# Vandermode/ELD

Measured on AMD Instinct MI355X. Metric: raw megapixels/sec (noise-synth + U-Net step), higher is better.
Workload: dtype f32; 1 GPU; BASELINE.json configs[1]: full ELD noise model (PGRU, SonyA7S2 params) on 4x1424x2128 packed raw + U-Net fp32 train step (fwd, L1, bwd, Adam), 8 frames per GPU; images_per_gpu=8, global_batch=8, parallelism=dp1

## Files before the change

eld_amd/csrc/conv_wgrad.hip:

```cpp
#include <stdlib.h>
#include "conv.h"

#define TW 32
#define JB 32

typedef __bf16 bf16x8 __attribute__((ext_vector_type(8)));
typedef short s16x4 __attribute__((ext_vector_type(4)));
typedef int i32x4_t __attribute__((ext_vector_type(4)));
typedef _Float16 half8 __attribute__((ext_vector_type(8)));

enum { ALG_F32 = 0, ALG_BFM = 1, ALG_X3 = 2, ALG_H2 = 3 };

template <typename T, int MODE, int WCO, int TH, int ALG>
__global__ __launch_bounds__(256, 2) void wgrad_kernel(const WgradArgs a) {
    constexpr bool BFM = ALG == ALG_BFM, X3 = ALG == ALG_X3, H2 = ALG == ALG_H2;
    static_assert(!(X3 || H2) || sizeof(T) == 4, "x3 / h2: fp32 inputs");
    constexpr int ES = sizeof(T);
    constexpr int EPU = 16 / ES;
    constexpr int LES = X3 ? 6 : (BFM ? 2 : 4);
    constexpr int TAPS = MODE == CONV_3X3 ? 9 : 4;
    constexpr int WPIX = 4 / WCO;
    constexpr int COB = 32 * WCO;
    constexpr int TPIX = TH * TW;
    constexpr int PW = TPIX / WPIX;
    constexpr int KS = PW / 2;
    constexpr int X_PIX = MODE == CONV_3X3 ? (TH + 2) * (TW + 2) : 4 * TPIX;
    extern __shared__ __attribute__((aligned(16))) float lds[];
    constexpr int GROWS = TPIX + ((X3 || H2) ? 1 : 0);
    float* ldsG = lds;
    float* ldsX = lds + GROWS * COB * LES / 4;

    const int tid = threadIdx.x, lane = tid & 63, wave = tid >> 6;
    const int m = lane & 31, hi = lane >> 5;
    const int wco = wave % WCO, wpix = wave / WCO;
    const int IB = a.CA / COB, JBn = a.CBp / JB;
    int bid = xcd_block(a.xcd);
    const int jb = bid % JBn; bid /= JBn;
    const int ib = bid % IB;
    const int ps = bid / IB;
    const int i0 = ib * COB, j0 = jb * JB;
// ... 254 lines not shown
                const int row = (i & 3) + 8 * (i >> 2) + 4 * hi;
                a.part[pbase + ((size_t)t * a.CA + i0 + wco * 32 + row) * a.CBp + j0 + m] = H2 ? acc[t][i] * (1.0f / sc_g) * (1.0f / sc_x) : acc[t][i];
            }
        }
    }
    if (a.bpart && jb == 0) {
        red[wave * 64 + lane] = bsum;
        __syncthreads();
        if (tid < COB) {
            const int wc = tid / 32, mm = tid % 32;
            float s = 0.f;
            for (int wp = 0; wp < WPIX; ++wp) s += red[(wp * WCO + wc) * 64 + mm] + red[(wp * WCO + wc) * 64 + 32 + mm];
            a.bpart[(size_t)ps * a.CA + i0 + tid] = H2 ? s * (1.0f / sc_g) : s;
        }
    }
    if constexpr (XSUM) {
        if (xsum_on) {
            __syncthreads();
            float* r = lds;
#pragma unroll
            for (int e = 0; e < EPU; ++e) r[tid * EPU + e] = xs[e];
            __syncthreads();
            if (tid < JB) {
                constexpr int PARTS = JB / EPU;
                const int part = tid / EPU, comp = tid % EPU;
                float s = 0.f;
                for (int k = 0; k < 256 / PARTS; ++k) s += r[(k * PARTS + part) * EPU + comp];
                a.xbpart[(size_t)ps * a.CBp + j0 + tid] = s;
            }
        }
    }
}

template <typename T, int WCO, int WCI, int WPIX, int TH, int TWT, int STREAM = 0>
__global__ __launch_bounds__(512, 2) void wgrad8_kernel(const WgradArgs a) {
    constexpr int ES = sizeof(T), EPU = 16 / ES, NPC = ES == 4 ? 3 : 1, XQ = 32 / EPU;
    static_assert(WCO * WCI * WPIX == 8, "8 waves");
    constexpr int THREADS = 512, TAPS = 9;
    constexpr int COB = 32 * WCO, JBK = 32 * WCI, TPIX = TH * TWT, PW = TPIX / WPIX, KSB = PW / 16;
    static_assert(TWT == 8 || TWT == 16 || TWT == 32, "tile width");
    static_assert(PW % 16 == 0 && PW >= 16, "a wave's pixel slice is a whole number of 16-pixel k-steps");
    constexpr int X_PIX = (TH + 2) * (TWT + 2);
    constexpr int GBLK = TPIX * 32 + (ES == 4 ? 32 : 0);
    constexpr int GPL = GBLK * WCO, XPL = X_PIX * JBK;
    constexpr int G_Q = COB / EPU, G_UNITS = TPIX * G_Q, G_IT = G_UNITS / THREADS;
    static_assert(G_UNITS % THREADS == 0 && THREADS % G_Q == 0, "a thread stages the same channel quad of G in every iteration");
    constexpr int X_UNITS1 = X_PIX * XQ, X_IT = (X_UNITS1 + THREADS - 1) / THREADS;
    extern __shared__ __attribute__((aligned(16))) float lds[];
    bf16_t* ldsG = reinterpret_cast<bf16_t*>(lds);
    bf16_t* ldsX = ldsG + NPC * GPL;

    const int tid = threadIdx.x, lane = tid & 63, wave = tid >> 6;
    const int m = lane & 31, hi = lane >> 5;
    const int wco = wave % WCO, wci = (wave / WCO) % WCI, wpix = wave / (WCO * WCI);
    const int IB = a.CA / COB, JBn = a.CBp / JBK;
    int bid = xcd_block(a.xcd);
    const int jb = bid % JBn; bid /= JBn;
    const int ib = bid % IB;
    const int ps = bid / IB;
    const int i0 = ib * COB, j0 = jb * JBK;
    const bool do_bias = a.bpart != nullptr && jb == 0;

    f32x16 acc[TAPS];
#pragma unroll
    for (int t = 0; t < TAPS; ++t)
#pragma unroll
        for (int i = 0; i < 16; ++i) acc[t][i] = 0.f;
    float4 bsum4 = make_float4(0.f, 0.f, 0.f, 0.f), bsum4b = make_float4(0.f, 0.f, 0.f, 0.f);

    const int ntiles = a.tiles_x * a.tiles_y;
    const int VP = a.vp;
    const bool seam = VP % TH != 0;
    constexpr unsigned OOB = 0xFFFFFFF0u;
    constexpr int G_STEP = THREADS / G_Q;
    const int g_part = tid % G_Q, g_lp0 = tid / G_Q;
    const int g_px0 = g_lp0 % TWT, g_py0 = g_lp0 / TWT;
    const unsigned g_off0 = (unsigned)(g_px0 * a.CA + i0 + g_part * EPU) * (unsigned)ES;
    const int g_lds0 = ((g_part * EPU) >> 5) * GBLK + g_lp0 * 32 + ((g_part * EPU) & 31);
    auto g_pxy = [&](int it, int& dpx, int& dpy) {
        if (G_STEP >= TWT) { dpx = 0; dpy = it * (G_STEP / TWT); }
        else { dpx = (it * G_STEP) % TWT; dpy = (it * G_STEP) / TWT; }
    };
    const int x_part = (int)((unsigned)tid % (unsigned)XQ);
    int x_hyx[X_IT];
#pragma unroll
    for (int it = 0; it < X_IT; ++it) {
        const int hp = (int)((unsigned)(tid + it * THREADS) / (unsigned)XQ);
        const int hy = hp / (TWT + 2);
        x_hyx[it] = (hy << 8) | (hp - hy * (TWT + 2));
    }
    auto x_alive = [&](int it) { return (it + 1) * THREADS <= X_UNITS1 || (int)((unsigned)(tid + it * THREADS) / (unsigned)XQ) < X_PIX; };
    const char* xs[WCI]; int xC[WCI], xc0[WCI];
#pragma unroll
    for (int cb = 0; cb < WCI; ++cb) {
        const int c = j0 + cb * 32;
        if (c < a.C0) { xs[cb] = static_cast<const char*>(a.x0); xC[cb] = a.C0; xc0[cb] = c; }
        else if (c < a.C0 + a.C1) { xs[cb] = static_cast<const char*>(a.x1); xC[cb] = a.C1; xc0[cb] = c - a.C0; }
        else { xs[cb] = nullptr; xC[cb] = 32; xc0[cb] = 0; }
    }
    float4 rg[G_IT], rx[WCI][X_IT];
// ... 68 lines not shown
        const unsigned y0 = __float_as_uint(r0), y1 = __float_as_uint(r1), y2 = __float_as_uint(r2), y3 = __float_as_uint(r3);
        const unsigned z0 = __float_as_uint(r0 - __uint_as_float(y0 & 0xFFFF0000u)), z1 = __float_as_uint(r1 - __uint_as_float(y1 & 0xFFFF0000u));
        const unsigned z2 = __float_as_uint(r2 - __uint_as_float(y2 & 0xFFFF0000u)), z3 = __float_as_uint(r3 - __uint_as_float(y3 & 0xFFFF0000u));
        auto hp = [](unsigned lo, unsigned hi_) { return __builtin_amdgcn_perm(hi_, lo, 0x07060302u); };
        *reinterpret_cast<uint2*>(d) = make_uint2(hp(x0, x1), hp(x2, x3));
        *reinterpret_cast<uint2*>(d + plane_elems) = make_uint2(hp(y0, y1), hp(y2, y3));
        *reinterpret_cast<uint2*>(d + 2 * plane_elems) = make_uint2(hp(z0, z1), hp(z2, z3));
    };
    auto store_tile = [&]() {
#pragma unroll
        for (int it = 0; it < G_IT; ++it) {
            put3(ldsG + g_lds0 + it * G_STEP * 32, GPL, rg[it]);
            if (do_bias) {
                if constexpr (ES == 4) { bsum4.x += rg[it].x; bsum4.y += rg[it].y; bsum4.z += rg[it].z; bsum4.w += rg[it].w; }
                else {
                    const uint4 q = __builtin_bit_cast(uint4, rg[it]);
                    const float4 lo = unpack_bf4(make_uint2(q.x, q.y)), hi4 = unpack_bf4(make_uint2(q.z, q.w));
                    bsum4.x += lo.x; bsum4.y += lo.y; bsum4.z += lo.z; bsum4.w += lo.w;
                    bsum4b.x += hi4.x; bsum4b.y += hi4.y; bsum4b.z += hi4.z; bsum4b.w += hi4.w;
                }
            }
        }
#pragma unroll
        for (int cb = 0; cb < WCI; ++cb)
#pragma unroll
            for (int it = 0; it < X_IT; ++it)
                if (x_alive(it)) put3(ldsX + (cb * X_PIX + (int)((unsigned)(tid + it * THREADS) / (unsigned)XQ)) * 32 + x_part * EPU, XPL, rx[cb][it]);
    };

    const int gi = lane & 15, gg = lane >> 4;
    constexpr bool ROWSHARE = STREAM == 2;
    static_assert(!ROWSHARE || (NPC == 3 && TWT == 8 && WPIX == 1 && TH % 2 == 0), "row-shared fragments: fp32, 8-pixel-wide tiles, one pixel slice");
    constexpr int HS = TH / 2;
    const int lq0 = ROWSHARE ? HS * TWT * hi + (gi >> 2) : wpix * PW + 8 * hi + (gi >> 2);
    const int pyq = lq0 / TWT, pxq = lq0 - pyq * TWT;
    const bf16_t* gq = ldsG + wco * GBLK + lq0 * 32 + (gg & 1) * 16 + (gi & 3) * 4;
    const bf16_t* xq = ldsX + (wci * X_PIX + pyq * (TWT + 2) + pxq) * 32 + (gg & 1) * 16 + (gi & 3) * 4;
    auto tr8 = [](const bf16_t* p0) {
        const s16x4 lo = __builtin_amdgcn_ds_read_tr16_b64_v4i16((__attribute__((address_space(3))) s16x4*)p0);
        const s16x4 hi4 = __builtin_amdgcn_ds_read_tr16_b64_v4i16((__attribute__((address_space(3))) s16x4*)(p0 + 4 * 32));
        return __builtin_bit_cast(bf16x8, __builtin_shufflevector(lo, hi4, 0, 1, 2, 3, 4, 5, 6, 7));
    };

    if (ps < ntiles) load_tile(ps);
    for (int tile = ps; tile < ntiles; tile += a.psplit) {
        __syncthreads();
        store_tile();
        __syncthreads();
        if (tile + a.psplit < ntiles) load_tile(tile + a.psplit);
        if constexpr (ROWSHARE) {
            constexpr int GI[6] = {0, 1, 2, 0, 1, 0};
            constexpr int XI[6] = {2, 1, 0, 1, 0, 0};
            constexpr int NU = (HS + 2) * 3;
            bf16x8 gr[3][3], xf[2][3];
            auto readG = [&](int s_, bf16x8 (&g3)[3]) {
#pragma unroll
                for (int pc = 0; pc < 3; ++pc) g3[pc] = tr8(gq + pc * GPL + s_ * TWT * 32);
            };
            auto readF = [&](int a_, int kx, bf16x8 (&x3)[3]) {
#pragma unroll
                for (int pc = 0; pc < 3; ++pc) x3[pc] = tr8(xq + pc * XPL + (a_ * (TWT + 2) + kx) * 32);
            };
            readG(0, gr[0]);
            readF(0, 0, xf[0]);
#pragma unroll
            for (int u = 0; u < NU; ++u) {
                const int a_ = u / 3, kx = u % 3;
                if (u + 1 < NU) readF((u + 1) / 3, (u + 1) % 3, xf[(u + 1) & 1]);
                __builtin_amdgcn_sched_barrier(0);
#pragma unroll
// ... 13 lines not shown
            }
        } else
        if constexpr (NPC == 3 && STREAM == 1) {
            constexpr int GI[6] = {0, 1, 2, 0, 1, 0};
            constexpr int XI[6] = {2, 1, 0, 1, 0, 0};
            constexpr int NBLK = KSB * TAPS;
            bf16x8 ga[2][3], xb[2][3];
            auto readG = [&](int ks, bf16x8 (&g3)[3]) {
#pragma unroll
                for (int pc = 0; pc < 3; ++pc) g3[pc] = tr8(gq + pc * GPL + ks * 16 * 32);
            };
            auto readX = [&](int ks, int t, bf16x8 (&x3)[3]) {
                const int lrel = ks * 16, dy0 = lrel / TWT, dxp = lrel - dy0 * TWT;
                const int xoff = (dy0 + t / 3) * (TWT + 2) + dxp + t % 3;
#pragma unroll
                for (int pc = 0; pc < 3; ++pc) x3[pc] = tr8(xq + pc * XPL + xoff * 32);
            };
            readG(0, ga[0]);
            readX(0, 0, xb[0]);
#pragma unroll
            for (int b = 0; b < NBLK; ++b) {
                const int ks = b / TAPS, t = b % TAPS;
                if (b + 1 < NBLK) {
                    const int ks1 = (b + 1) / TAPS, t1 = (b + 1) % TAPS;
                    readX(ks1, t1, xb[(b + 1) & 1]);
                    if (ks1 != ks) readG(ks1, ga[ks1 & 1]);
                }
                __builtin_amdgcn_sched_barrier(0);
#pragma unroll
                for (int q = 0; q < 6; ++q) acc[t] = __builtin_amdgcn_mfma_f32_32x32x16_bf16(ga[ks & 1][GI[q]], xb[b & 1][XI[q]], acc[t], 0, 0, 0);
                __builtin_amdgcn_sched_barrier(0);
            }
        } else
#pragma unroll
        for (int ks = 0; ks < KSB; ++ks) {
            const int lrel = ks * 16;
            const int dy0 = lrel / TWT, dxp = lrel - dy0 * TWT;
            bf16x8 ga[NPC];
#pragma unroll
            for (int pc = 0; pc < NPC; ++pc) ga[pc] = tr8(gq + pc * GPL + lrel * 32);
#pragma unroll
            for (int t0 = 0; t0 < TAPS; t0 += 3) {
                bf16x8 xb[3][NPC];
#pragma unroll
                for (int tt = 0; tt < 3; ++tt) {
                    const int xoff = (dy0 + t0 / 3) * (TWT + 2) + dxp + tt;
#pragma unroll
                    for (int pc = 0; pc < NPC; ++pc) xb[tt][pc] = tr8(xq + pc * XPL + xoff * 32);
                }
                if constexpr (NPC == 3) {
                    constexpr int GI[6] = {0, 1, 2, 0, 1, 0};
                    constexpr int XI[6] = {2, 1, 0, 1, 0, 0};
#pragma unroll
                    for (int q = 0; q < 6; ++q)
#pragma unroll
                        for (int tt = 0; tt < 3; ++tt)
                            acc[t0 + tt] = __builtin_amdgcn_mfma_f32_32x32x16_bf16(ga[GI[q]], xb[tt][XI[q]], acc[t0 + tt], 0, 0, 0);
                } else {
#pragma unroll
                    for (int tt = 0; tt < 3; ++tt) acc[t0 + tt] = __builtin_amdgcn_mfma_f32_32x32x16_bf16(ga[0], xb[tt][0], acc[t0 + tt], 0, 0, 0);
                }
                __builtin_amdgcn_sched_barrier(0);
            }
        }
    }

    __syncthreads();
    float* red = lds;
    const size_t pbase = (size_t)ps * TAPS * a.CA * a.CBp;
    const int wt = wci * WCO + wco;
#pragma unroll
    for (int t = 0; t < TAPS; ++t) {
        if (WPIX > 1) {
            if (wpix > 0) {
#pragma unroll
                for (int i = 0; i < 16; ++i) red[(((wpix - 1) * (WCO * WCI) + wt) * 16 + i) * 64 + lane] = acc[t][i];
            }
            __syncthreads();
            if (wpix == 0) {
                for (int w = 0; w < WPIX - 1; ++w)
#pragma unroll
                    for (int i = 0; i < 16; ++i) acc[t][i] += red[((w * (WCO * WCI) + wt) * 16 + i) * 64 + lane];
            }
            __syncthreads();
        }
        if (wpix == 0) {
#pragma unroll
            for (int i = 0; i < 16; ++i) {
                const int row = (i & 3) + 8 * (i >> 2) + 4 * hi;
                a.part[pbase + ((size_t)t * a.CA + i0 + wco * 32 + row) * a.CBp + j0 + wci * 32 + m] = acc[t][i];
            }
        }
    }
    if (do_bias) {
        __syncthreads();
        if constexpr (ES == 4) reinterpret_cast<float4*>(red)[tid] = bsum4;
        else { reinterpret_cast<float4*>(red)[2 * tid] = bsum4; reinterpret_cast<float4*>(red)[2 * tid + 1] = bsum4b; }
        __syncthreads();
        if (tid < COB) {
            const int q = tid / EPU, comp = tid % EPU;
            float s_ = 0.f;
            for (int k = 0; k < THREADS / G_Q; ++k) s_ += red[(q + k * G_Q) * EPU + comp];
            a.bpart[(size_t)ps * a.CA + i0 + tid] = s_;
        }
    }
}

__device__ __forceinline__ void wg_dma16(i32x4_t rsrc, unsigned voff, unsigned lds_dst) {
    unsigned keep;
    asm volatile("s_nop 4\n\ts_mov_b32 %0, m0\n\ts_mov_b32 m0, %3\n\ts_nop 0\n\tbuffer_load_dwordx4 %1, %2, 0 offen lds\n\ts_mov_b32 m0, %0"
                 : "=&s"(keep) : "v"(voff), "s"(rsrc), "s"(lds_dst) : "memory");
}

template <int WCO, int WCI, int WPIX, int TH, int TWT>
__global__ __launch_bounds__(512, 2) void wgrad8d_kernel(const WgradArgs a) {
    static_assert(WCO * WCI * WPIX == 8, "8 waves");
    static_assert(TWT == 8 || TWT == 16 || TWT == 32, "tile width");
    constexpr int WAVES = 8, THREADS = 512, TAPS = 9;
    constexpr int COB = 32 * WCO, JBK = 32 * WCI, TPIX = TH * TWT, PW = TPIX / WPIX, KSB = PW / 16;
    static_assert(PW % 16 == 0 && PW >= 16, "a wave's pixel slice is a whole number of 16-pixel k-steps");
    constexpr int HW = TWT + 2, X_PIX = (TH + 2) * HW;
    static_assert((TPIX * 4) % 64 == 0, "a block of G is whole DMA pieces");
    constexpr int GB_PIECES = TPIX * 4 / 64, XB_PIECES = (X_PIX * 4 + 63) / 64;
// ... 169 lines not shown
            __syncthreads();
            if (wpix == 0) {
                for (int w = 0; w < WPIX - 1; ++w)
#pragma unroll
                    for (int i = 0; i < 16; ++i) acc[t][i] += red[((w * (WCO * WCI) + wt) * 16 + i) * 64 + lane];
            }
            __syncthreads();
        }
        if (wpix == 0) {
#pragma unroll
            for (int i = 0; i < 16; ++i) {
                const int row = (i & 3) + 8 * (i >> 2) + 4 * hi;
                a.part[pbase + ((size_t)t * a.CA + i0 + wco * 32 + row) * a.CBp + j0 + wci * 32 + m] = acc[t][i];
            }
        }
    }
    if (do_bias) {
        __syncthreads();
        reinterpret_cast<float4*>(red)[2 * tid] = bsum4; reinterpret_cast<float4*>(red)[2 * tid + 1] = bsum4b;
        __syncthreads();
        if (tid < COB) {
            const int q = tid / 8, comp = tid % 8;
            float s_ = 0.f;
            for (int k = 0; k < THREADS / G_Q; ++k) s_ += red[(q + k * G_Q) * 8 + comp];
            a.bpart[(size_t)ps * a.CA + i0 + tid] = s_;
        }
    }
}

static int wgrad8_dma() {
    static const int on = [] { const char* e = getenv("ELD_WGRAD_DMA"); return e ? (int)(atoi(e) != 0) : 1; }();
    return on && !(debug_kernel_mask(-1) & 16);
}
template <int DUMMY>
__global__ __launch_bounds__(512, 2) void wgradt8_kernel(const WgradArgs a) {
    constexpr int WCO = 4, WCI = 2, TH = 8, TWT = 8, TPIX = TH * TWT, THREADS = 512, TAPS = 4, NPC = 3;
    constexpr int COB = 32 * WCO, JBK = 32 * WCI, KSB = TPIX / 16;
    constexpr int GBLK = TPIX * 32 + 32;
    constexpr int GPL = GBLK * WCO, X_PIX = TAPS * TPIX, XPL = X_PIX * JBK;
    constexpr int G_IT = TPIX * (COB / 4) / THREADS, X_IT = X_PIX * 8 / THREADS;
    extern __shared__ __attribute__((aligned(16))) float lds[];
    bf16_t* ldsG = reinterpret_cast<bf16_t*>(lds);
    bf16_t* ldsX = ldsG + NPC * GPL;
    const int tid = threadIdx.x, lane = tid & 63, wave = tid >> 6;
    const int m = lane & 31, hi = lane >> 5;
    const int wco = wave % WCO, wci = wave / WCO;
    const int IB = a.CA / COB, JBn = a.CBp / JBK;
    int bid = xcd_block(a.xcd);
    const int jb = bid % JBn; bid /= JBn;
    const int ib = bid % IB;
    const int ps = bid / IB;
    const int i0 = ib * COB, j0 = jb * JBK;
    const bool xsum_on = a.xbpart != nullptr && ib == 0;
    const int Wx = 2 * a.W, CB = a.C0;

    f32x16 acc[TAPS];
#pragma unroll
    for (int t = 0; t < TAPS; ++t)
#pragma unroll
        for (int i = 0; i < 16; ++i) acc[t][i] = 0.f;
    float4 xs4[WCI];
#pragma unroll
    for (int cb = 0; cb < WCI; ++cb) xs4[cb] = make_float4(0.f, 0.f, 0.f, 0.f);

    const int tiles_per_img = a.tiles_x * a.tiles_y, ntiles = tiles_per_img * a.N;
    constexpr unsigned OOB = 0xFFFFFFF0u;
    const int g_part = tid & 31, g_lp0 = tid >> 5, x_part = tid & 7, x_lp = tid >> 3;
    const int x_py = x_lp / TWT, x_px = x_lp - x_py * TWT;
    float4 rg[G_IT], rx[WCI][X_IT];
    const size_t g_img = (size_t)a.H * a.W * a.CA * 4, x_img = (size_t)4 * a.H * a.W * CB * 4;
    auto load_tile = [&](int tile) {
        const int img = tile / tiles_per_img;
        int ty, tx;
        band_tile(tile - img * tiles_per_img, a.tiles_x, a.tiles_y, a.band, ty, tx);
        const int y0 = ty * TH, x0 = tx * TWT;
        const __amdgpu_buffer_rsrc_t rs_g = __builtin_amdgcn_make_buffer_rsrc((void*)(static_cast<const char*>(a.g) + (size_t)img * g_img), 0, (int)g_img, 0x00020000);
        const __amdgpu_buffer_rsrc_t rs_x = __builtin_amdgcn_make_buffer_rsrc((void*)(static_cast<const char*>(a.x0) + (size_t)img * x_img), 0, (int)x_img, 0x00020000);
#pragma unroll
        for (int it = 0; it < G_IT; ++it) {
            const int lp = g_lp0 + 16 * it, py = lp / TWT, px = lp - py * TWT;
            const int gy = y0 + py, gx = x0 + px;
            const unsigned off = (gy < a.H && gx < a.W) ? (unsigned)(((gy * a.W + gx) * a.CA + i0 + g_part * 4) * 4) : OOB;
            rg[it] = __builtin_bit_cast(float4, __builtin_amdgcn_raw_buffer_load_b128(rs_g, (int)off, 0, 0));
        }
        const bool pok = y0 + x_py < a.H && x0 + x_px < a.W;
#pragma unroll
        for (int cb = 0; cb < WCI; ++cb)
#pragma unroll
            for (int it = 0; it < X_IT; ++it) {
                const int gy = 2 * (y0 + x_py) + (it >> 1), gx = 2 * (x0 + x_px) + (it & 1);
                const unsigned off = pok ? (unsigned)(((gy * Wx + gx) * CB + j0 + cb * 32 + x_part * 4) * 4) : OOB;
                rx[cb][it] = __builtin_bit_cast(float4, __builtin_amdgcn_raw_buffer_load_b128(rs_x, (int)off, 0, 0));
            }
    };
    auto put3 = [&](bf16_t* d, int plane_elems, const float4& raw) {
        const unsigned x0 = __float_as_uint(raw.x), x1 = __float_as_uint(raw.y), x2 = __float_as_uint(raw.z), x3 = __float_as_uint(raw.w);
        const float r0 = raw.x - __uint_as_float(x0 & 0xFFFF0000u), r1 = raw.y - __uint_as_float(x1 & 0xFFFF0000u);
        const float r2 = raw.z - __uint_as_float(x2 & 0xFFFF0000u), r3 = raw.w - __uint_as_float(x3 & 0xFFFF0000u);
        const unsigned y0 = __float_as_uint(r0), y1 = __float_as_uint(r1), y2 = __float_as_uint(r2), y3 = __float_as_uint(r3);
        const unsigned z0 = __float_as_uint(r0 - __uint_as_float(y0 & 0xFFFF0000u)), z1 = __float_as_uint(r1 - __uint_as_float(y1 & 0xFFFF0000u));
        const unsigned z2 = __float_as_uint(r2 - __uint_as_float(y2 & 0xFFFF0000u)), z3 = __float_as_uint(r3 - __uint_as_float(y3 & 0xFFFF0000u));
        auto hp = [](unsigned lo, unsigned hi_) { return __builtin_amdgcn_perm(hi_, lo, 0x07060302u); };
        *reinterpret_cast<uint2*>(d) = make_uint2(hp(x0, x1), hp(x2, x3));
        *reinterpret_cast<uint2*>(d + plane_elems) = make_uint2(hp(y0, y1), hp(y2, y3));
        *reinterpret_cast<uint2*>(d + 2 * plane_elems) = make_uint2(hp(z0, z1), hp(z2, z3));
    };
    auto store_tile = [&]() {
#pragma unroll
        for (int it = 0; it < G_IT; ++it)
            put3(ldsG + ((g_part * 4) >> 5) * GBLK + (g_lp0 + 16 * it) * 32 + ((g_part * 4) & 31), GPL, rg[it]);
#pragma unroll
        for (int cb = 0; cb < WCI; ++cb)
#pragma unroll
            for (int it = 0; it < X_IT; ++it) {
                put3(ldsX + (cb * X_PIX + it * TPIX + x_lp) * 32 + x_part * 4, XPL, rx[cb][it]);
                if (xsum_on) { xs4[cb].x += rx[cb][it].x; xs4[cb].y += rx[cb][it].y; xs4[cb].z += rx[cb][it].z; xs4[cb].w += rx[cb][it].w; }
            }
    };
    const int gi = lane & 15, gg = lane >> 4;
    const int lq0 = 8 * hi + (gi >> 2);
    const bf16_t* gq = ldsG + wco * GBLK + lq0 * 32 + (gg & 1) * 16 + (gi & 3) * 4;
    const bf16_t* xq = ldsX + (wci * X_PIX + lq0) * 32 + (gg & 1) * 16 + (gi & 3) * 4;
    auto tr8 = [](const bf16_t* p0) {
        const s16x4 lo = __builtin_amdgcn_ds_read_tr16_b64_v4i16((__attribute__((address_space(3))) s16x4*)p0);
        const s16x4 hi4 = __builtin_amdgcn_ds_read_tr16_b64_v4i16((__attribute__((address_space(3))) s16x4*)(p0 + 4 * 32));
        return __builtin_bit_cast(bf16x8, __builtin_shufflevector(lo, hi4, 0, 1, 2, 3, 4, 5, 6, 7));
    };

    if (ps < ntiles) load_tile(ps);
    for (int tile = ps; tile < ntiles; tile += a.psplit) {
        __syncthreads();
        store_tile();
        __syncthreads();
        if (tile + a.psplit < ntiles) load_tile(tile + a.psplit);
#pragma unroll
        for (int ks = 0; ks < KSB; ++ks) {
            bf16x8 ga[NPC];
#pragma unroll
            for (int pc = 0; pc < NPC; ++pc) ga[pc] = tr8(gq + pc * GPL + ks * 16 * 32);
#pragma unroll
            for (int t0 = 0; t0 < TAPS; t0 += 2) {
                bf16x8 xb[2][NPC];
#pragma unroll
                for (int tt = 0; tt < 2; ++tt)
#pragma unroll
                    for (int pc = 0; pc < NPC; ++pc) xb[tt][pc] = tr8(xq + pc * XPL + ((t0 + tt) * TPIX + ks * 16) * 32);
                constexpr int GI[6] = {0, 1, 2, 0, 1, 0};
                constexpr int XI[6] = {2, 1, 0, 1, 0, 0};
#pragma unroll
                for (int q = 0; q < 6; ++q)
#pragma unroll
                    for (int tt = 0; tt < 2; ++tt)
                        acc[t0 + tt] = __builtin_amdgcn_mfma_f32_32x32x16_bf16(ga[GI[q]], xb[tt][XI[q]], acc[t0 + tt], 0, 0, 0);
            }
        }
    }
    const size_t pbase = (size_t)ps * TAPS * a.CA * a.CBp;
#pragma unroll
    for (int t = 0; t < TAPS; ++t)
#pragma unroll
        for (int i = 0; i < 16; ++i) {
            const int row = (i & 3) + 8 * (i >> 2) + 4 * hi;
            a.part[pbase + ((size_t)t * a.CA + i0 + wco * 32 + row) * a.CBp + j0 + wci * 32 + m] = acc[t][i];
        }
    if (xsum_on) {
        __syncthreads();
        float4* r = reinterpret_cast<float4*>(lds);
#pragma unroll
        for (int cb = 0; cb < WCI; ++cb) r[cb * THREADS + tid] = xs4[cb];
        __syncthreads();
        if (tid < JBK) {
            const int cb = tid >> 5, c = tid & 31, quad = c >> 2, comp = c & 3;
            float s_ = 0.f;
            for (int k = 0; k < THREADS / 8; ++k) s_ += reinterpret_cast<const float*>(&r[cb * THREADS + quad + 8 * k])[comp];
            a.xbpart[(size_t)ps * a.CBp + j0 + tid] = s_;
        }
    }
}

bool wgradt8_takes(int CA, int CB) {
    static const int on = [] { const char* e = getenv("ELD_WGRADT8"); return e ? atoi(e) : 1; }();
    return on && CA % 128 == 0 && CB % 64 == 0;
}
int wgradt8_ntiles(int N, int H, int W) { return ((W + 7) / 8) * ((H + 7) / 8) * N; }

static int launch_wt8(WgradArgs a, hipStream_t st) {
    eld_note_conv_kernel("wgradt8");
    a.xcd = eld_xcd_mask() & XCD_WGRAD8;
    a.band = eld_tile_band();
    a.tiles_x = (a.W + 7) / 8;
    a.tiles_y = (a.H + 7) / 8;
    const size_t lds_bytes = (size_t)(3 * 4 * (64 * 32 + 32) + 3 * 2 * 256 * 32) * 2;
    const long long blocks = (long long)(a.CA / 128) * (a.CBp / 64) * a.psplit;
    if (blocks <= 0) return 0;
    if ((size_t)4 * a.H * a.W * a.C0 * 4 >= 0xFFFFFFF0ull || (size_t)a.H * a.W * a.CA * 4 >= 0xFFFFFFF0ull) return ELD_ENOTSUP;
    auto kern = wgradt8_kernel<0>;
    static EldAttrOnce once;
    { const int rc = once.ensure(kern, lds_bytes); if (rc) return rc; }
    ELD_LAUNCH(kern, dim3((unsigned)blocks), dim3(512), lds_bytes, st, a);
    ELD_LAUNCH_CHECK();
    return 0;
}

bool wgrad8_shape(int CA, int CBp, int& COB, int& JBK, int& TH, int& TWo, bool bf16) {
    if (CA % 32 || CBp % 32) return false;
    TWo = 32;
    if (CA % 128 == 0 && CBp % 64 == 0) { COB = 128; JBK = 64; TH = 2; }
    else if (CA % 64 == 0 && CBp % 64 == 0) { COB = 64; JBK = 64; TH = 2; }
    else if (CA % 64 == 0) { COB = 64; JBK = 32; TH = 4; }
    else if (CBp % 64 == 0) { COB = 32; JBK = 64; TH = 4; }
    else { COB = 32; JBK = 32; TH = 4; }
    if (bf16) TH = 8;
    if (bf16 && wgrad8_dma() && COB == 128) { TH = 16; TWo = 8; return true; }
    if (COB == 128) { TH = TH * 4; TWo = 8; }
    return true;
}

int wgrad8_ntiles(int CA, int CBp, int N, int H, int W, bool bf16) {
    int COB, JBK, TH, TWo;
    if (!wgrad8_shape(CA, CBp, COB, JBK, TH, TWo, bf16)) return 0;
    const int VP = vrow_pitch(N, H, TH);
    return ((W + TWo - 1) / TWo) * ((vrow_extent(N, H, VP) + TH - 1) / TH);
}

template <typename T, int WCO, int WCI, int WPIX, int TH, int TWT, int STREAM = 0>
static int launch_w8(WgradArgs a, hipStream_t st) {
    a.xcd = eld_xcd_mask() & XCD_WGRAD8;
    a.band = eld_tile_band();
    constexpr int COB = 32 * WCO, JBK = 32 * WCI;
    eld_note_conv_variant(sizeof(T) == 2 ? "wgrad8<bf16>" : (COB == 128 ? "wgrad8<f32,128x64>" : (COB == 64 ? (JBK == 64 ? "wgrad8<f32,64x64>" : "wgrad8<f32,64x32>")
                                                                                                     : (JBK == 64 ? "wgrad8<f32,32x64>" : "wgrad8<f32,32x32>"))),
                          STREAM == 1 ? "stream" : (STREAM == 2 ? "rowshare" : nullptr));
    a.vp = vrow_pitch(a.N, a.H, TH);
    a.tiles_x = (a.W + TWT - 1) / TWT;
    a.tiles_y = (vrow_extent(a.N, a.H, a.vp) + TH - 1) / TH;
    size_t lds_bytes = (size_t)((TH * TWT * 32 + (sizeof(T) == 4 ? 32 : 0)) * (COB / 32) + (TH + 2) * (TWT + 2) * JBK) * (sizeof(T) == 4 ? 6 : 2);
    const size_t red_bytes = (size_t)7 * 16 * 64 * sizeof(float) * 1;
    if (lds_bytes < red_bytes) lds_bytes = red_bytes;
    const long long blocks = (long long)(a.CA / COB) * (a.CBp / JBK) * a.psplit;
    if (blocks <= 0) return 0;
    auto kern = wgrad8_kernel<T, WCO, WCI, WPIX, TH, TWT, STREAM>;
    static EldAttrOnce once;
    { const int rc = once.ensure(kern, lds_bytes); if (rc) return rc; }
    ELD_LAUNCH(kern, dim3((unsigned)blocks), dim3(512), lds_bytes, st, a);
    ELD_LAUNCH_CHECK();
    return 0;
}

template <int WCO, int WCI, int WPIX, int TH, int TWT>
static int launch_w8d(WgradArgs a, hipStream_t st) {
    eld_note_conv_kernel("wgrad8d");
    a.xcd = eld_xcd_mask() & XCD_WGRAD8;
    a.band = eld_tile_band();
    constexpr int COB = 32 * WCO, JBK = 32 * WCI;
    a.vp = vrow_pitch(a.N, a.H, TH);
    a.tiles_x = (a.W + TWT - 1) / TWT;
    a.tiles_y = (vrow_extent(a.N, a.H, a.vp) + TH - 1) / TH;
    constexpr int PIECES = WCO * (TH * TWT * 4 / 64) + WCI * (((TH + 2) * (TWT + 2) * 4 + 63) / 64);
    size_t lds_bytes = (size_t)2 * PIECES * 1024;
    const size_t red_bytes = (size_t)7 * 16 * 64 * sizeof(float);
    if (lds_bytes < red_bytes) lds_bytes = red_bytes;
    const long long blocks = (long long)(a.CA / COB) * (a.CBp / JBK) * a.psplit;
    if (blocks <= 0) return 0;
    auto kern = wgrad8d_kernel<WCO, WCI, WPIX, TH, TWT>;
    static EldAttrOnce once;
    { const int rc = once.ensure(kern, lds_bytes); if (rc) return rc; }
    ELD_LAUNCH(kern, dim3((unsigned)blocks), dim3(512), lds_bytes, st, a);
    ELD_LAUNCH_CHECK();
    return 0;
}

static int launch_wgrad8(const WgradArgs& a, hipStream_t st) {
    const bool bf16 = a.dtype == DT_BF16;
    const size_t es = bf16 ? 2 : 4;
    int COB, JBK, TH, TWo;
    if (!wgrad8_shape(a.CA, a.CBp, COB, JBK, TH, TWo, bf16)) return ELD_ENOTSUP;
    if ((a.C0 % 32) || (a.C1 % 32)) return ELD_ENOTSUP;
    const size_t win = a.N > 1 ? 2 : 1;
    if ((size_t)a.H * a.W * a.CA * es * win >= 0xFFFFFFF0ull || (size_t)a.H * a.W * (a.C0 > a.C1 ? a.C0 : a.C1) * es * win >= 0xFFFFFFF0ull) return ELD_ENOTSUP;
    if (bf16 && wgrad8_dma() && COB == 128) {
        return launch_w8d<4, 2, 1, 16, 8>(a, st);
    }
    if (bf16) {
        if (COB == 128) return launch_w8<bf16_t, 4, 2, 1, 32, 8>(a, st);
        if (COB == 64 && JBK == 64) return launch_w8<bf16_t, 2, 2, 2, 8, 32>(a, st);
        if (COB == 64) return launch_w8<bf16_t, 2, 1, 4, 8, 32>(a, st);
        if (JBK == 64) return launch_w8<bf16_t, 1, 2, 4, 8, 32>(a, st);
        return launch_w8<bf16_t, 1, 1, 8, 8, 32>(a, st);
    }
    static const int stream = [] { const char* e = getenv("ELD_WG8_STREAM"); return e ? atoi(e) : 0; }();
    static const int rowshare = [] { const char* e = getenv("ELD_WG8_ROWSHARE"); return e ? atoi(e) : 0; }();
    if (COB == 128 && rowshare) return launch_w8<float, 4, 2, 1, 8, 8, 2>(a, st);
    if (COB == 128) return (stream & 1) ? launch_w8<float, 4, 2, 1, 8, 8, 1>(a, st) : launch_w8<float, 4, 2, 1, 8, 8>(a, st);
    if (stream & 2) {
        if (COB == 64 && JBK == 64) return launch_w8<float, 2, 2, 2, 2, 32, 1>(a, st);
        if (COB == 64) return launch_w8<float, 2, 1, 4, 4, 32, 1>(a, st);
        if (JBK == 64) return launch_w8<float, 1, 2, 4, 4, 32, 1>(a, st);
        return launch_w8<float, 1, 1, 8, 4, 32, 1>(a, st);
    }
    if (COB == 64 && JBK == 64) return launch_w8<float, 2, 2, 2, 2, 32>(a, st);
    if (COB == 64) return launch_w8<float, 2, 1, 4, 4, 32>(a, st);
    if (JBK == 64) return launch_w8<float, 1, 2, 4, 4, 32>(a, st);
    return launch_w8<float, 1, 1, 8, 4, 32>(a, st);
}

template <typename T, int MODE, int WCO, int TH, int ALG = ALG_F32>
static int launch_w(WgradArgs a, hipStream_t st) {
    eld_note_conv_variant(sizeof(T) == 2 ? (MODE == CONV_3X3 ? "wgrad<bf16>" : "wgrad<bf16,gather>") : (MODE == CONV_3X3 ? "wgrad<f32>" : "wgrad<f32,gather>"),
                          (sizeof(T) == 2 && ALG == ALG_F32) ? "f32mma" : nullptr);
    a.xcd = eld_xcd_mask() & XCD_WGRAD;
    constexpr int COB = 32 * WCO;
    constexpr int X_PIX = MODE == CONV_3X3 ? (TH + 2) * (TW + 2) : 4 * TH * TW;
    a.tiles_x = (a.W + TW - 1) / TW;
    a.tiles_y = (a.H + TH - 1) / TH;
    constexpr int GROWS = TH * TW + ((ALG == ALG_X3 || ALG == ALG_H2) ? 1 : 0);
    size_t lds_bytes = (size_t)(GROWS * COB + X_PIX * JB) * (ALG == ALG_X3 ? 6 : (ALG == ALG_BFM ? 2 : 4));
    const size_t red_bytes = (size_t)4 * 16 * 64 * sizeof(float);
    if (lds_bytes < red_bytes) lds_bytes = red_bytes;
    const long long blocks = (long long)(a.CA / COB) * (a.CBp / JB) * a.psplit;
    if (blocks <= 0) return 0;
    auto kern = wgrad_kernel<T, MODE, WCO, TH, ALG>;
    static EldAttrOnce once;
    { const int rc = once.ensure(kern, lds_bytes); if (rc) return rc; }
    ELD_LAUNCH(kern, dim3((unsigned)blocks), dim3(256), lds_bytes, st, a);
    ELD_LAUNCH_CHECK();
    return 0;
}

int launch_wgrad(const WgradArgs& a, int mode, hipStream_t st) {
    if (a.CA % 32 || a.CBp % 32 || a.C0 % 4 || a.C1 % 4 || a.psplit < 1) return ELD_EINVAL;
    if (a.C1 > 0 && a.C0 % 32) return ELD_EINVAL;
    const bool c64 = a.CA % 64 == 0;
    if (a.dtype == DT_BF16) {
        if (a.C0 % 8 || a.C1 % 8) return ELD_EINVAL;
        if (mode == CONV_3X3 && a.wgrad8) {
            const int rc = launch_wgrad8(a, st);
            if (rc != ELD_ENOTSUP) return rc;
        }
        static const int mma = [] { const char* e = getenv("ELD_WGRAD_BF16_MMA"); return e ? atoi(e) : 1; }();
        if (mma) {
            if (mode == CONV_3X3) return c64 ? launch_w<bf16_t, CONV_3X3, 2, 4, ALG_BFM>(a, st) : launch_w<bf16_t, CONV_3X3, 1, 4, ALG_BFM>(a, st);
            if (mode == CONV_GATHER2X2) return c64 ? launch_w<bf16_t, CONV_GATHER2X2, 2, 2, ALG_BFM>(a, st) : launch_w<bf16_t, CONV_GATHER2X2, 1, 2, ALG_BFM>(a, st);
            return ELD_EINVAL;
        }
        if (mode == CONV_3X3) return c64 ? launch_w<bf16_t, CONV_3X3, 2, 4>(a, st) : launch_w<bf16_t, CONV_3X3, 1, 4>(a, st);
        if (mode == CONV_GATHER2X2) return c64 ? launch_w<bf16_t, CONV_GATHER2X2, 2, 2>(a, st) : launch_w<bf16_t, CONV_GATHER2X2, 1, 2>(a, st);
        return ELD_EINVAL;
    }
    const int algo = resolve_algo(a.algo);
    if (algo == 2) {
        if (!a.amax_g || !a.amax_x0) return ELD_EINVAL;
        if (mode == CONV_3X3) return c64 ? launch_w<float, CONV_3X3, 2, 2, ALG_H2>(a, st) : launch_w<float, CONV_3X3, 1, 4, ALG_H2>(a, st);
        if (mode == CONV_GATHER2X2) return c64 ? launch_w<float, CONV_GATHER2X2, 2, 2, ALG_H2>(a, st) : launch_w<float, CONV_GATHER2X2, 1, 2, ALG_H2>(a, st);
        return ELD_EINVAL;
    }
    if (mode == CONV_3X3 && algo == 1 && a.wgrad8) {
        const int rc = launch_wgrad8(a, st);
        if (rc != ELD_ENOTSUP) return rc;
    }
    if (mode == CONV_3X3 && algo == 1) return c64 ? launch_w<float, CONV_3X3, 2, 2, ALG_X3>(a, st) : launch_w<float, CONV_3X3, 1, 2, ALG_X3>(a, st);
    if (mode == CONV_3X3) return c64 ? launch_w<float, CONV_3X3, 2, 4>(a, st) : launch_w<float, CONV_3X3, 1, 4>(a, st);
    if (mode == CONV_GATHER2X2 && algo == 1 && a.wgrad8 && a.C1 == 0 && a.C0 == a.CBp && wgradt8_takes(a.CA, a.C0)) return launch_wt8(a, st);
    if (mode == CONV_GATHER2X2 && algo == 1) return c64 ? launch_w<float, CONV_GATHER2X2, 2, 2, ALG_X3>(a, st) : launch_w<float, CONV_GATHER2X2, 1, 2, ALG_X3>(a, st);
    if (mode == CONV_GATHER2X2) return c64 ? launch_w<float, CONV_GATHER2X2, 2, 2>(a, st) : launch_w<float, CONV_GATHER2X2, 1, 2>(a, st);
    return ELD_EINVAL;
}

template <int T>
__global__ __launch_bounds__(1024) void wgrad_reduce_kernel(const float* __restrict__ part, const float* __restrict__ bpart, float* __restrict__ wgrad,
                                                            float* __restrict__ bgrad, int psplit, int CA, int CBp, int CBr, int pair_blocks, int NB) {
    extern __shared__ float sh[];
    const int lane = threadIdx.x & 63, w = threadIdx.x >> 6, NW = blockDim.x >> 6;
    const size_t pairs = (size_t)CA * CBp, plane = pairs * T;
    if ((int)blockIdx.x >= pair_blocks) {
        const int c = ((int)blockIdx.x - pair_blocks) * 64 + lane;
        float b = 0.f;
        if (c < NB) {
            int k = w;
            for (; k + 3 * NW < psplit; k += 4 * NW)
                b += (bpart[(size_t)k * NB + c] + bpart[(size_t)(k + NW) * NB + c]) + (bpart[(size_t)(k + 2 * NW) * NB + c] + bpart[(size_t)(k + 3 * NW) * NB + c]);
            for (; k < psplit; k += NW) b += bpart[(size_t)k * NB + c];
        }
        sh[w * 64 + lane] = b;
        __syncthreads();
        if (w == 0 && c < NB) {
            for (int ww = 1; ww < NW; ++ww) b += sh[ww * 64 + lane];
            bgrad[c] = b;
        }
        return;
    }
    const size_t pr = (size_t)blockIdx.x * 64 + lane;
    float s[T];
#pragma unroll
    for (int t = 0; t < T; ++t) s[t] = 0.f;
    if (pr < pairs) {
// ... 51 lines not shown
```

Measured before the change: 741.5 raw MPix/s.

## Use 16x16x32 bf16 MFMA tiles in wgrad8 and wgradt8 weight-gradient kernels

```diff
diff --git a/eld_amd/csrc/conv_wgrad.hip b/eld_amd/csrc/conv_wgrad.hip
--- a/eld_amd/csrc/conv_wgrad.hip
+++ b/eld_amd/csrc/conv_wgrad.hip
@@ -6,6 +6,7 @@
 
 typedef __bf16 bf16x8 __attribute__((ext_vector_type(8)));
 typedef short s16x4 __attribute__((ext_vector_type(4)));
+typedef float f32x4 __attribute__((ext_vector_type(4)));
 typedef int i32x4_t __attribute__((ext_vector_type(4)));
 typedef _Float16 half8 __attribute__((ext_vector_type(8)));
 
@@ -326,7 +327,7 @@
     }
 }
 
-template <typename T, int WCO, int WCI, int WPIX, int TH, int TWT, int STREAM = 0>
+template <typename T, int WCO, int WCI, int WPIX, int TH, int TWT, int STREAM = 0, int MF = 32>
 __global__ __launch_bounds__(512, 2) void wgrad8_kernel(const WgradArgs a) {
     constexpr int ES = sizeof(T), EPU = 16 / ES, NPC = ES == 4 ? 3 : 1, XQ = 32 / EPU;
     static_assert(WCO * WCI * WPIX == 8, "8 waves");
@@ -334,6 +335,8 @@
     constexpr int COB = 32 * WCO, JBK = 32 * WCI, TPIX = TH * TWT, PW = TPIX / WPIX, KSB = PW / 16;
     static_assert(TWT == 8 || TWT == 16 || TWT == 32, "tile width");
     static_assert(PW % 16 == 0 && PW >= 16, "a wave's pixel slice is a whole number of 16-pixel k-steps");
+    static_assert(MF == 32 || (MF == 16 && NPC == 3 && STREAM == 0 && PW % 32 == 0), "16x16x32 products: fp32 inputs, the plain loop, whole 32-pixel k-steps");
+    constexpr bool M16 = MF == 16;
     constexpr int X_PIX = (TH + 2) * (TWT + 2);
     constexpr int GBLK = TPIX * 32 + (ES == 4 ? 32 : 0);
     constexpr int GPL = GBLK * WCO, XPL = X_PIX * JBK;
@@ -355,11 +358,15 @@
     const int i0 = ib * COB, j0 = jb * JBK;
     const bool do_bias = a.bpart != nullptr && jb == 0;
 
-    f32x16 acc[TAPS];
+    f32x16 acc[M16 ? 1 : TAPS];
+    f32x4 acc4[M16 ? TAPS : 1][4];
 #pragma unroll
     for (int t = 0; t < TAPS; ++t)
 #pragma unroll
-        for (int i = 0; i < 16; ++i) acc[t][i] = 0.f;
+        for (int i = 0; i < 16; ++i) {
+            if constexpr (M16) acc4[t][i >> 2][i & 3] = 0.f;
+            else acc[t][i] = 0.f;
+        }
     float4 bsum4 = make_float4(0.f, 0.f, 0.f, 0.f), bsum4b = make_float4(0.f, 0.f, 0.f, 0.f);
 
     const int ntiles = a.tiles_x * a.tiles_y;
@@ -494,10 +501,11 @@
     constexpr bool ROWSHARE = STREAM == 2;
     static_assert(!ROWSHARE || (NPC == 3 && TWT == 8 && WPIX == 1 && TH % 2 == 0), "row-shared fragments: fp32, 8-pixel-wide tiles, one pixel slice");
     constexpr int HS = TH / 2;
-    const int lq0 = ROWSHARE ? HS * TWT * hi + (gi >> 2) : wpix * PW + 8 * hi + (gi >> 2);
+    const int lq0 = ROWSHARE ? HS * TWT * hi + (gi >> 2) : wpix * PW + 8 * (M16 ? gg : hi) + (gi >> 2);
     const int pyq = lq0 / TWT, pxq = lq0 - pyq * TWT;
-    const bf16_t* gq = ldsG + wco * GBLK + lq0 * 32 + (gg & 1) * 16 + (gi & 3) * 4;
-    const bf16_t* xq = ldsX + (wci * X_PIX + pyq * (TWT + 2) + pxq) * 32 + (gg & 1) * 16 + (gi & 3) * 4;
+    const int chq = M16 ? 0 : (gg & 1) * 16;
+    const bf16_t* gq = ldsG + wco * GBLK + lq0 * 32 + chq + (gi & 3) * 4;
+    const bf16_t* xq = ldsX + (wci * X_PIX + pyq * (TWT + 2) + pxq) * 32 + chq + (gi & 3) * 4;
     auto tr8 = [](const bf16_t* p0) {
         const s16x4 lo = __builtin_amdgcn_ds_read_tr16_b64_v4i16((__attribute__((address_space(3))) s16x4*)p0);
         const s16x4 hi4 = __builtin_amdgcn_ds_read_tr16_b64_v4i16((__attribute__((address_space(3))) s16x4*)(p0 + 4 * 32));
@@ -577,6 +585,43 @@
                 __builtin_amdgcn_sched_barrier(0);
             }
         } else
+        if constexpr (M16) {
+            constexpr int GI[6] = {0, 1, 2, 0, 1, 0};
+            constexpr int XI[6] = {2, 1, 0, 1, 0, 0};
+            constexpr int UPK = TAPS * 2, NU = (KSB / 2) * UPK;
+            bf16x8 ga[3][2], xb[3];
+            auto readG = [&](int ks, int pc) {
+#pragma unroll
+                for (int h = 0; h < 2; ++h) ga[pc][h] = tr8(gq + pc * GPL + ks * 32 * 32 + h * 16);
+            };
+            auto readX = [&](int u, int pc) {
+                const int lrel = (u / UPK) * 32, t = (u % UPK) / 2, nh = u % 2;
+                const int dy0 = lrel / TWT, dxp = lrel - dy0 * TWT;
+                const int xoff = (dy0 + t / 3) * (TWT + 2) + dxp + t % 3;
+                xb[pc] = tr8(xq + pc * XPL + xoff * 32 + nh * 16);
+            };
+            __builtin_amdgcn_sched_barrier(0);
+#pragma unroll
+            for (int pc = 0; pc < 3; ++pc) readG(0, pc);
+#pragma unroll
+            for (int pc = 2; pc >= 0; --pc) readX(0, pc);
+#pragma unroll
+            for (int u = 0; u < NU; ++u) {
+                const int t = (u % UPK) / 2, nh = u % 2;
+                const bool nxt = u + 1 < NU, newk = nxt && (u + 1) % UPK == 0;
+#pragma unroll
+                for (int q = 0; q < 6; ++q) {
+                    __builtin_amdgcn_sched_barrier(0);
+#pragma unroll
+                    for (int mh = 0; mh < 2; ++mh)
+                        acc4[t][2 * mh + nh] = __builtin_amdgcn_mfma_f32_16x16x32_bf16(ga[GI[q]][mh], xb[XI[q]], acc4[t][2 * mh + nh], 0, 0, 0);
+                    __builtin_amdgcn_sched_barrier(0);
+                    if (nxt && (q == 0 || q == 3 || q == 5)) readX(u + 1, q == 0 ? 2 : (q == 3 ? 1 : 0));
+                    if (newk && (q == 2 || q == 4 || q == 5)) readG((u + 1) / UPK, q == 2 ? 2 : (q == 4 ? 1 : 0));
+                }
+            }
+            __builtin_amdgcn_sched_barrier(0);
+        } else
 #pragma unroll
         for (int ks = 0; ks < KSB; ++ks) {
             const int lrel = ks * 16;
@@ -616,24 +661,31 @@
     const int wt = wci * WCO + wco;
 #pragma unroll
     for (int t = 0; t < TAPS; ++t) {
+        float av[16];
+#pragma unroll
+        for (int i = 0; i < 16; ++i) {
+            if constexpr (M16) av[i] = acc4[t][i >> 2][i & 3];
+            else av[i] = acc[t][i];
+        }
         if (WPIX > 1) {
             if (wpix > 0) {
 #pragma unroll
-                for (int i = 0; i < 16; ++i) red[(((wpix - 1) * (WCO * WCI) + wt) * 16 + i) * 64 + lane] = acc[t][i];
+                for (int i = 0; i < 16; ++i) red[(((wpix - 1) * (WCO * WCI) + wt) * 16 + i) * 64 + lane] = av[i];
             }
             __syncthreads();
             if (wpix == 0) {
                 for (int w = 0; w < WPIX - 1; ++w)
 #pragma unroll
-                    for (int i = 0; i < 16; ++i) acc[t][i] += red[((w * (WCO * WCI) + wt) * 16 + i) * 64 + lane];
+                    for (int i = 0; i < 16; ++i) av[i] += red[((w * (WCO * WCI) + wt) * 16 + i) * 64 + lane];
             }
             __syncthreads();
         }
         if (wpix == 0) {
 #pragma unroll
             for (int i = 0; i < 16; ++i) {
-                const int row = (i & 3) + 8 * (i >> 2) + 4 * hi;
-                a.part[pbase + ((size_t)t * a.CA + i0 + wco * 32 + row) * a.CBp + j0 + wci * 32 + m] = acc[t][i];
+                const int row = M16 ? 16 * (i >> 3) + 4 * gg + (i & 3) : (i & 3) + 8 * (i >> 2) + 4 * hi;
+                const int col = M16 ? 16 * ((i >> 2) & 1) + gi : m;
+                a.part[pbase + ((size_t)t * a.CA + i0 + wco * 32 + row) * a.CBp + j0 + wci * 32 + col] = av[i];
             }
         }
     }
@@ -869,7 +921,7 @@
     static const int on = [] { const char* e = getenv("ELD_WGRAD_DMA"); return e ? (int)(atoi(e) != 0) : 1; }();
     return on && !(debug_kernel_mask(-1) & 16);
 }
-template <int DUMMY>
+template <int M16>
 __global__ __launch_bounds__(512, 2) void wgradt8_kernel(const WgradArgs a) {
     constexpr int WCO = 4, WCI = 2, TH = 8, TWT = 8, TPIX = TH * TWT, THREADS = 512, TAPS = 4, NPC = 3;
     constexpr int COB = 32 * WCO, JBK = 32 * WCI, KSB = TPIX / 16;
@@ -891,11 +943,15 @@
     const bool xsum_on = a.xbpart != nullptr && ib == 0;
     const int Wx = 2 * a.W, CB = a.C0;
 
-    f32x16 acc[TAPS];
+    f32x16 acc[M16 ? 1 : TAPS];
+    f32x4 acc4[M16 ? TAPS : 1][4];
 #pragma unroll
     for (int t = 0; t < TAPS; ++t)
 #pragma unroll
-        for (int i = 0; i < 16; ++i) acc[t][i] = 0.f;
+        for (int i = 0; i < 16; ++i) {
+            if constexpr (M16) acc4[t][i >> 2][i & 3] = 0.f;
+            else acc[t][i] = 0.f;
+        }
     float4 xs4[WCI];
 #pragma unroll
     for (int cb = 0; cb < WCI; ++cb) xs4[cb] = make_float4(0.f, 0.f, 0.f, 0.f);
@@ -955,9 +1011,10 @@
             }
     };
     const int gi = lane & 15, gg = lane >> 4;
-    const int lq0 = 8 * hi + (gi >> 2);
-    const bf16_t* gq = ldsG + wco * GBLK + lq0 * 32 + (gg & 1) * 16 + (gi & 3) * 4;
-    const bf16_t* xq = ldsX + (wci * X_PIX + lq0) * 32 + (gg & 1) * 16 + (gi & 3) * 4;
+    const int lq0 = 8 * (M16 ? gg : hi) + (gi >> 2);
+    const int chq = M16 ? 0 : (gg & 1) * 16;
+    const bf16_t* gq = ldsG + wco * GBLK + lq0 * 32 + chq + (gi & 3) * 4;
+    const bf16_t* xq = ldsX + (wci * X_PIX + lq0) * 32 + chq + (gi & 3) * 4;
     auto tr8 = [](const bf16_t* p0) {
         const s16x4 lo = __builtin_amdgcn_ds_read_tr16_b64_v4i16((__attribute__((address_space(3))) s16x4*)p0);
         const s16x4 hi4 = __builtin_amdgcn_ds_read_tr16_b64_v4i16((__attribute__((address_space(3))) s16x4*)(p0 + 4 * 32));
@@ -970,6 +1027,38 @@
         store_tile();
         __syncthreads();
         if (tile + a.psplit < ntiles) load_tile(tile + a.psplit);
+        if constexpr (M16) {
+            constexpr int GI[6] = {0, 1, 2, 0, 1, 0};
+            constexpr int XI[6] = {2, 1, 0, 1, 0, 0};
+            constexpr int UPK = TAPS * 2, NU = (KSB / 2) * UPK;
+            bf16x8 ga[NPC][2], xb[NPC];
+            auto readG = [&](int ks, int pc) {
+#pragma unroll
+                for (int h = 0; h < 2; ++h) ga[pc][h] = tr8(gq + pc * GPL + ks * 32 * 32 + h * 16);
+            };
+            auto readX = [&](int u, int pc) { xb[pc] = tr8(xq + pc * XPL + (((u % UPK) / 2) * TPIX + (u / UPK) * 32) * 32 + (u % 2) * 16); };
+            __builtin_amdgcn_sched_barrier(0);
+#pragma unroll
+            for (int pc = 0; pc < NPC; ++pc) readG(0, pc);
+#pragma unroll
+            for (int pc = NPC - 1; pc >= 0; --pc) readX(0, pc);
+#pragma unroll
+            for (int u = 0; u < NU; ++u) {
+                const int t = (u % UPK) / 2, nh = u % 2;
+                const bool nxt = u + 1 < NU, newk = nxt && (u + 1) % UPK == 0;
+#pragma unroll
+                for (int q = 0; q < 6; ++q) {
+                    __builtin_amdgcn_sched_barrier(0);
+#pragma unroll
+                    for (int mh = 0; mh < 2; ++mh)
+                        acc4[t][2 * mh + nh] = __builtin_amdgcn_mfma_f32_16x16x32_bf16(ga[GI[q]][mh], xb[XI[q]], acc4[t][2 * mh + nh], 0, 0, 0);
+                    __builtin_amdgcn_sched_barrier(0);
+                    if (nxt && (q == 0 || q == 3 || q == 5)) readX(u + 1, q == 0 ? 2 : (q == 3 ? 1 : 0));
+                    if (newk && (q == 2 || q == 4 || q == 5)) readG((u + 1) / UPK, q == 2 ? 2 : (q == 4 ? 1 : 0));
+                }
+            }
+            __builtin_amdgcn_sched_barrier(0);
+        } else
 #pragma unroll
         for (int ks = 0; ks < KSB; ++ks) {
             bf16x8 ga[NPC];
@@ -997,8 +1086,12 @@
     for (int t = 0; t < TAPS; ++t)
 #pragma unroll
         for (int i = 0; i < 16; ++i) {
-            const int row = (i & 3) + 8 * (i >> 2) + 4 * hi;
-            a.part[pbase + ((size_t)t * a.CA + i0 + wco * 32 + row) * a.CBp + j0 + wci * 32 + m] = acc[t][i];
+            const int row = M16 ? 16 * (i >> 3) + 4 * gg + (i & 3) : (i & 3) + 8 * (i >> 2) + 4 * hi;
+            const int col = M16 ? 16 * ((i >> 2) & 1) + gi : m;
+            float v;
+            if constexpr (M16) v = acc4[t][i >> 2][i & 3];
+            else v = acc[t][i];
+            a.part[pbase + ((size_t)t * a.CA + i0 + wco * 32 + row) * a.CBp + j0 + wci * 32 + col] = v;
         }
     if (xsum_on) {
         __syncthreads();
@@ -1021,8 +1114,15 @@
 }
 int wgradt8_ntiles(int N, int H, int W) { return ((W + 7) / 8) * ((H + 7) / 8) * N; }
 
+#ifndef ELD_WG_MF16
+#define ELD_WG_MF16 15
+#endif
+enum { WG_MF_128x64 = 1, WG_MF_64x64 = 2, WG_MF_32x64 = 4, WG_MF_64x32 = 8, WG_MF_T8 = 16 };
+static bool wg_mf16_on() { return !(debug_kernel_mask(-1) & 512); }
+
+template <int M16>
 static int launch_wt8(WgradArgs a, hipStream_t st) {
-    eld_note_conv_kernel("wgradt8");
+    eld_note_conv_variant("wgradt8", (!M16 && (ELD_WG_MF16 & WG_MF_T8)) ? "mfma32" : nullptr);
     a.xcd = eld_xcd_mask() & XCD_WGRAD8;
     a.band = eld_tile_band();
     a.tiles_x = (a.W + 7) / 8;
@@ -1031,7 +1131,7 @@
     const long long blocks = (long long)(a.CA / 128) * (a.CBp / 64) * a.psplit;
     if (blocks <= 0) return 0;
     if ((size_t)4 * a.H * a.W * a.C0 * 4 >= 0xFFFFFFF0ull || (size_t)a.H * a.W * a.CA * 4 >= 0xFFFFFFF0ull) return ELD_ENOTSUP;
-    auto kern = wgradt8_kernel<0>;
+    auto kern = wgradt8_kernel<M16>;
     static EldAttrOnce once;
     { const int rc = once.ensure(kern, lds_bytes); if (rc) return rc; }
     ELD_LAUNCH(kern, dim3((unsigned)blocks), dim3(512), lds_bytes, st, a);
@@ -1060,14 +1160,16 @@
     return ((W + TWo - 1) / TWo) * ((vrow_extent(N, H, VP) + TH - 1) / TH);
 }
 
-template <typename T, int WCO, int WCI, int WPIX, int TH, int TWT, int STREAM = 0>
+template <typename T, int WCO, int WCI, int WPIX, int TH, int TWT, int STREAM = 0, int MF = 32>
 static int launch_w8(WgradArgs a, hipStream_t st) {
     a.xcd = eld_xcd_mask() & XCD_WGRAD8;
     a.band = eld_tile_band();
     constexpr int COB = 32 * WCO, JBK = 32 * WCI;
+    constexpr int MFBIT = COB == 128 ? WG_MF_128x64 : (COB == 64 ? (JBK == 64 ? WG_MF_64x64 : WG_MF_64x32) : (JBK == 64 ? WG_MF_32x64 : 0));
     eld_note_conv_variant(sizeof(T) == 2 ? "wgrad8<bf16>" : (COB == 128 ? "wgrad8<f32,128x64>" : (COB == 64 ? (JBK == 64 ? "wgrad8<f32,64x64>" : "wgrad8<f32,64x32>")
                                                                                                      : (JBK == 64 ? "wgrad8<f32,32x64>" : "wgrad8<f32,32x32>"))),
-                          STREAM == 1 ? "stream" : (STREAM == 2 ? "rowshare" : nullptr));
+                          STREAM == 1 ? "stream" : (STREAM == 2 ? "rowshare" : nullptr),
+                          (sizeof(T) == 4 && STREAM == 0 && MF == 32 && (ELD_WG_MF16 & MFBIT)) ? "mfma32" : nullptr);
     a.vp = vrow_pitch(a.N, a.H, TH);
     a.tiles_x = (a.W + TWT - 1) / TWT;
     a.tiles_y = (vrow_extent(a.N, a.H, a.vp) + TH - 1) / TH;
@@ -1076,7 +1178,7 @@
     if (lds_bytes < red_bytes) lds_bytes = red_bytes;
     const long long blocks = (long long)(a.CA / COB) * (a.CBp / JBK) * a.psplit;
     if (blocks <= 0) return 0;
-    auto kern = wgrad8_kernel<T, WCO, WCI, WPIX, TH, TWT, STREAM>;
+    auto kern = wgrad8_kernel<T, WCO, WCI, WPIX, TH, TWT, STREAM, MF>;
     static EldAttrOnce once;
     { const int rc = once.ensure(kern, lds_bytes); if (rc) return rc; }
     ELD_LAUNCH(kern, dim3((unsigned)blocks), dim3(512), lds_bytes, st, a);
@@ -1128,13 +1230,26 @@
     static const int stream = [] { const char* e = getenv("ELD_WG8_STREAM"); return e ? atoi(e) : 0; }();
     static const int rowshare = [] { const char* e = getenv("ELD_WG8_ROWSHARE"); return e ? atoi(e) : 0; }();
     if (COB == 128 && rowshare) return launch_w8<float, 4, 2, 1, 8, 8, 2>(a, st);
-    if (COB == 128) return (stream & 1) ? launch_w8<float, 4, 2, 1, 8, 8, 1>(a, st) : launch_w8<float, 4, 2, 1, 8, 8>(a, st);
+    if (COB == 128 && (stream & 1)) return launch_w8<float, 4, 2, 1, 8, 8, 1>(a, st);
+#if ELD_WG_MF16 & 1
+    if (COB == 128 && wg_mf16_on()) return launch_w8<float, 4, 2, 1, 8, 8, 0, 16>(a, st);
+#endif
+    if (COB == 128) return launch_w8<float, 4, 2, 1, 8, 8>(a, st);
     if (stream & 2) {
         if (COB == 64 && JBK == 64) return launch_w8<float, 2, 2, 2, 2, 32, 1>(a, st);
         if (COB == 64) return launch_w8<float, 2, 1, 4, 4, 32, 1>(a, st);
         if (JBK == 64) return launch_w8<float, 1, 2, 4, 4, 32, 1>(a, st);
         return launch_w8<float, 1, 1, 8, 4, 32, 1>(a, st);
     }
+#if ELD_WG_MF16 & 2
+    if (COB == 64 && JBK == 64 && wg_mf16_on()) return launch_w8<float, 2, 2, 2, 2, 32, 0, 16>(a, st);
+#endif
+#if ELD_WG_MF16 & 8
+    if (COB == 64 && JBK == 32 && wg_mf16_on()) return launch_w8<float, 2, 1, 4, 4, 32, 0, 16>(a, st);
+#endif
+#if ELD_WG_MF16 & 4
+    if (COB == 32 && JBK == 64 && wg_mf16_on()) return launch_w8<float, 1, 2, 4, 4, 32, 0, 16>(a, st);
+#endif
     if (COB == 64 && JBK == 64) return launch_w8<float, 2, 2, 2, 2, 32>(a, st);
     if (COB == 64) return launch_w8<float, 2, 1, 4, 4, 32>(a, st);
     if (JBK == 64) return launch_w8<float, 1, 2, 4, 4, 32>(a, st);
@@ -1197,7 +1312,12 @@
     }
     if (mode == CONV_3X3 && algo == 1) return c64 ? launch_w<float, CONV_3X3, 2, 2, ALG_X3>(a, st) : launch_w<float, CONV_3X3, 1, 2, ALG_X3>(a, st);
     if (mode == CONV_3X3) return c64 ? launch_w<float, CONV_3X3, 2, 4>(a, st) : launch_w<float, CONV_3X3, 1, 4>(a, st);
-    if (mode == CONV_GATHER2X2 && algo == 1 && a.wgrad8 && a.C1 == 0 && a.C0 == a.CBp && wgradt8_takes(a.CA, a.C0)) return launch_wt8(a, st);
+    if (mode == CONV_GATHER2X2 && algo == 1 && a.wgrad8 && a.C1 == 0 && a.C0 == a.CBp && wgradt8_takes(a.CA, a.C0)) {
+#if ELD_WG_MF16 & 16
+        if (wg_mf16_on()) return launch_wt8<1>(a, st);
+#endif
+        return launch_wt8<0>(a, st);
+    }
     if (mode == CONV_GATHER2X2 && algo == 1) return c64 ? launch_w<float, CONV_GATHER2X2, 2, 2, ALG_X3>(a, st) : launch_w<float, CONV_GATHER2X2, 1, 2, ALG_X3>(a, st);
     if (mode == CONV_GATHER2X2) return c64 ? launch_w<float, CONV_GATHER2X2, 2, 2>(a, st) : launch_w<float, CONV_GATHER2X2, 1, 2>(a, st);
     return ELD_EINVAL;
```

Result: no change. 746.8 raw MPix/s, median of 6 (+0.7%).
